# KerkDovan/univer-ocr

Hardware: NVIDIA B200
Metric: my_model inference images/sec (page tiles through Monochrome->Paragraph + Line + Char forward) (higher is better)
Workload: dtype tf32/f32

## Files before the change

univer_ocr_b200/csrc/conv_pair_rows_tc.cu:

```cuda
#include <cuda.h>

#include "conv_common.cuh"
#include "tc_ptx.cuh"

namespace uocr {

int make_tmap_plain_tf32(CUtensorMap* map, const void* base, int rank, const uint64_t* dims,
                         const uint64_t* strides_bytes, const uint32_t* box);

namespace {

constexpr int PR_THREADS = 672;
constexpr int PR_RING = 8;
constexpr int PR_SLOT = 2048;
constexpr int PR_OUT = 246;
constexpr int PR_TSLOTS = 4;
constexpr int PR_LAG = 2;

struct PairRowsParams {
    const float* w1; const float* b1; const float* w2; const float* b2; float* y;
    int N, H, W;
    int xt, nb, rb, npair;
    int total;
    float alpha1, alpha2;
};

struct __align__(128) PairRowsSmem {
    float ring[(PR_RING + 1) * PR_SLOT / 4];
    float ones[128 * 4];
    float b1[2][10 * 64 * 4];
    float b2[4][256];
    float xch[2][2][2];
    uint64_t full[PR_RING], empty[PR_RING];
    uint64_t hfull[PR_TSLOTS], a2full[PR_TSLOTS], zfull[PR_TSLOTS], zempty[PR_TSLOTS];
    uint64_t drain;
    uint32_t tmem;
};

struct WorkUnit {
    int y0, rows;
    int t, n0, n1;
    int S, c0;
};

__device__ __forceinline__ WorkUnit pr_decode(const PairRowsParams& p, int w) {
    WorkUnit u;
    const int pi = w % p.npair;
    const int rest = w / p.npair;
    u.t = rest % p.xt;
    const int b = rest / p.xt;
    u.y0 = b * p.rb;
    u.rows = min(p.rb, p.H - u.y0);
    u.n0 = 2 * pi;
    u.n1 = 2 * pi + 1;
    u.c0 = (u.t & 1) ? 5 : 3;
    u.S = PR_OUT * u.t - 1 - u.c0;
    return u;
}

__device__ __forceinline__ void pr_wait(uint32_t bar, uint32_t parity) { mbar_wait(bar, parity); }

__device__ __forceinline__ void pr_ld16(uint32_t taddr, float* v) {
    uint32_t* r = reinterpret_cast<uint32_t*>(v);
    tc_ld16_nowait(taddr, r);
}
__device__ __forceinline__ void pr_st16(uint32_t taddr, const float* v) {
    tc_st16_nowait(taddr, reinterpret_cast<const uint32_t*>(v));
}

__device__ __forceinline__ bool pr_elect() {
    uint32_t pred;
    asm volatile("{\n\t.reg .pred p;\n\telect.sync _|p, 0xffffffff;\n\tselp.u32 %0, 1, 0, p;\n\t}" : "=r"(pred));
    return pred != 0;
}

__device__ void pr_producer(const PairRowsParams& p, const CUtensorMap* map, PairRowsSmem& sm) {
    const uint32_t ring = smem_u32(sm.ring);
    uint32_t ut = 0;
    for (int w = blockIdx.x; w < p.total; w += gridDim.x) {
        const WorkUnit u = pr_decode(p, w);
        const int nin = u.rows + 4;
        for (int r = 0; r < nin; ++r, ++ut) {
            const uint32_t slot = ut % PR_RING;
            pr_wait(smem_u32(&sm.empty[slot]), ((ut / PR_RING) & 1u) ^ 1u);
            if (pr_elect()) {
                const uint32_t bar = smem_u32(&sm.full[slot]);
                const bool mirror = slot == 0;
                mbar_arrive_expect_tx(bar, mirror ? 2u * PR_SLOT : (uint32_t)PR_SLOT);
                const int y = u.y0 - 2 + r;
                const uint32_t dst = ring + slot * PR_SLOT;
                tma_load_3d(dst, map, bar, u.S, y, u.n0);
                tma_load_3d(dst + 1024, map, bar, u.S, y, u.n1);
                if (mirror) {
                    const uint32_t dst2 = ring + PR_RING * PR_SLOT;
                    tma_load_3d(dst2, map, bar, u.S, y, u.n0);
                    tma_load_3d(dst2 + 1024, map, bar, u.S, y, u.n1);
                }
            }
            __syncwarp();
        }
    }
}

__device__ __forceinline__ void pr_conv2(PairRowsSmem& sm, uint32_t tmem, int j, uint32_t kv, uint64_t db2_0,
                                         uint64_t db2_1, uint32_t id16) {
    const uint32_t par = (kv / PR_TSLOTS) & 1u;
    pr_wait(smem_u32(&sm.a2full[j]), par);
    pr_wait(smem_u32(&sm.zempty[j]), par ^ 1u);
    tc_fence_after();
    if (pr_elect()) {
        const uint32_t base = tmem + 128u * (uint32_t)j;
#pragma unroll
        for (int f = 0; f < 4; ++f) {
            tc_mma_tf32_ts(base + 64u + 16u * f, base + 16u * f, db2_0 + 64u * f, id16, 0);
            tc_mma_tf32_ts(base + 64u + 16u * f, base + 16u * f + 8u, db2_1 + 64u * f, id16, 1);
        }
        tc_commit(smem_u32(&sm.zfull[j]));
    }
    __syncwarp();
}

__device__ void pr_mma(const PairRowsParams& p, PairRowsSmem& sm, uint32_t tmem, int j) {
    const uint32_t ring = smem_u32(sm.ring), ones = smem_u32(sm.ones), sb2 = smem_u32(sm.b2);
    const uint32_t id64 = (1u << 4) | (2u << 7) | (2u << 10) | ((64u >> 3) << 17) | ((128u >> 4) << 24);
    const uint32_t id16 = (1u << 4) | (2u << 7) | (2u << 10) | ((16u >> 3) << 17) | ((128u >> 4) << 24);
    const uint64_t da_row = make_kmajor_nosw_desc(0, 16, 128);
    const uint64_t da_pair = make_kmajor_nosw_desc(0, PR_SLOT, 128);
    const uint64_t da_bias = make_kmajor_nosw_desc(0, 0, 128);
    const uint64_t db2_0 = make_kmajor_nosw_desc(sb2, 256, 128), db2_1 = make_kmajor_nosw_desc(sb2 + 512, 256, 128);
    const uint32_t d1 = tmem + 128u * (uint32_t)j;
    uint32_t ut = 0, kv = 0;
    bool pending = false;
    uint32_t pkv = 0;
    for (int w = blockIdx.x; w < p.total; w += gridDim.x) {
        const WorkUnit u = pr_decode(p, w);
        const uint32_t sb1 = smem_u32(sm.b1[u.c0 == 5 ? 1 : 0]);
        const uint64_t db_ky0 = make_kmajor_nosw_desc(sb1 + 0 * 1024, 1024, 128);
        const uint64_t db_ky1 = make_kmajor_nosw_desc(sb1 + 3 * 1024, 1024, 128);
        const uint64_t db_ky2 = make_kmajor_nosw_desc(sb1 + 6 * 1024, 1024, 128);
        const uint64_t db_c2 = make_kmajor_nosw_desc(sb1 + 2 * 1024, 3 * 1024, 128);
        const uint64_t db_bias = make_kmajor_nosw_desc(sb1 + 8 * 1024, 1024, 128);
        const int nh = u.rows + 2;
        const int r_lo = u.y0 == 0 ? 1 : 0, r_hi = min(nh, p.H - u.y0 + 1);
        const int below = (j == 0 && r_hi < nh) ? r_hi : nh;
        int first = r_lo + (int)((uint32_t)(j - (int)(kv & 3u)) & 3u);
        if (first >= r_hi) first = below;
        int r = (j == 0 && r_lo == 1) ? 0 : first;
        while (r < nh) {
            const bool valid = r >= r_lo && r < r_hi;
            const uint32_t kvr = kv + (uint32_t)(r - r_lo);
            int r_next = r < r_lo ? first : (valid ? r + 4 : nh);
            if (valid && r_next >= r_hi) r_next = below;
            if (pending) {
                pr_conv2(sm, tmem, j, pkv, db2_0, db2_1, id16);
                pending = false;
            }
            const uint32_t u0 = ut + (uint32_t)r;
            const uint32_t s0 = u0 % PR_RING, s1 = (u0 + 1u) % PR_RING, s2 = (u0 + 2u) % PR_RING;
            const uint32_t e0 = smem_u32(&sm.empty[s0]), e1 = smem_u32(&sm.empty[s1]), e2 = smem_u32(&sm.empty[s2]);
            pr_wait(smem_u32(&sm.full[s0]), (u0 / PR_RING) & 1u);
            pr_wait(smem_u32(&sm.full[s1]), ((u0 + 1u) / PR_RING) & 1u);
            pr_wait(smem_u32(&sm.full[s2]), ((u0 + 2u) / PR_RING) & 1u);
            tc_fence_after();
            if (pr_elect()) {
                if (valid) {
                    const uint64_t a0 = (uint64_t)((ring + s0 * PR_SLOT) >> 4);
                    const uint64_t a1 = (uint64_t)((ring + s1 * PR_SLOT) >> 4);
                    const uint64_t a2 = (uint64_t)((ring + s2 * PR_SLOT) >> 4);
                    tc_mma_tf32(d1, da_row + a0, db_ky0, id64, 0);
                    tc_mma_tf32(d1, da_row + a1, db_ky1, id64, 1);
                    tc_mma_tf32(d1, da_row + a2, db_ky2, id64, 1);
                    tc_mma_tf32(d1, da_pair + a0 + 2u, db_c2, id64, 1);
                    tc_mma_tf32(d1, da_bias + (a2 + 2u) + ((uint64_t)((ones >> 4) - (uint32_t)(a2 + 2u)) << 16), db_bias,
                                id64, 1);
                    tc_commit(smem_u32(&sm.hfull[j]));
                    tc_commit(e0);
                    tc_commit(e1);
                    tc_commit(e2);
                } else {
                    mbar_arrive(e0);
                    mbar_arrive(e1);
                    mbar_arrive(e2);
                }
                if (r == 0) { mbar_arrive(e0); mbar_arrive(e0); mbar_arrive(e1); }
                if (r == nh - 1) { mbar_arrive(e1); mbar_arrive(e2); mbar_arrive(e2); }
            }
            __syncwarp();
            if (valid) { pending = true; pkv = kvr; }
            r = r_next;
        }
        kv += (uint32_t)(r_hi - r_lo);
        ut += (uint32_t)(nh + 2);
    }
    if (pending) pr_conv2(sm, tmem, j, pkv, db2_0, db2_1, id16);
    if (pr_elect()) tc_commit(smem_u32(&sm.drain));
    __syncwarp();
    pr_wait(smem_u32(&sm.drain), 0);
}

__device__ __forceinline__ int pr_tap(int f, int n) {
    int kx = -1, ky = 0;
    if (f == 0)      { if (n < 6) { kx = n / 3; ky = n % 3; } else if (n >= 8 && n < 11) { kx = 2; ky = n - 8; } }
    else if (f == 1) { if (n < 6) { kx = 1 + n / 3; ky = n % 3; } else if (n >= 8 && n < 11) { kx = 0; ky = n - 8; } }
    else if (f == 2) { if (n < 3) { kx = 2; ky = n; } else if (n >= 8 && n < 14) { kx = (n - 8) / 3; ky = (n - 8) % 3; } }
    else             { if (n < 3) { kx = 0; ky = n; } else if (n >= 8 && n < 14) { kx = 1 + (n - 8) / 3; ky = (n - 8) % 3; } }
    return kx < 0 ? -1 : ky * 3 + kx;
}

template <bool LEAKY>
__device__ void pr_act(const PairRowsParams& p, PairRowsSmem& sm, uint32_t tmem, int q, int type, int lane) {
    const uint32_t tl = tmem + ((uint32_t)(q * 32) << 16) + 32u * (uint32_t)type;
    const int j = (q & 1) * 32 + lane;
    const uint32_t hbar = smem_u32(&sm.hfull[0]), abar = smem_u32(&sm.a2full[0]);
    const uint32_t alpha_bits = __float_as_uint(p.alpha1);
    uint32_t k = 0;
    for (int w = blockIdx.x; w < p.total; w += gridDim.x) {
        const WorkUnit u = pr_decode(p, w);
        const int x0 = u.S + u.c0 + 4 * j + 2 * type;
        const bool in0 = x0 >= 0 && x0 < p.W, in1 = x0 + 1 >= 0 && x0 + 1 < p.W;
        const bool edge = !(in0 && in1);
        const int r_lo = u.y0 == 0 ? 1 : 0, r_hi = min(u.rows + 2, p.H - u.y0 + 1);
        for (int r = r_lo; r < r_hi; ++r, ++k) {
            const uint32_t s = k & 3u;
            pr_wait(hbar + 8u * s, (k >> 2) & 1u);
            tc_fence_after();
            uint32_t h[32];
            tc_ld16_nowait(tl + 128u * s, h);
            tc_ld16_nowait(tl + 128u * s + 16u, h + 16);
            tc_wait_ld();
            if (LEAKY) {
#pragma unroll
                for (int c = 0; c < 32; c += 2) {
                    uint32_t t0, t1;
                    asm("{\n\t.reg .b64 x, y, r;\n\tmov.b64 x, {%2, %3};\n\tmov.b64 y, {%4, %4};\n\t"
                        "mul.rn.f32x2 r, x, y;\n\tmov.b64 {%0, %1}, r;\n\t}"
                        : "=r"(t0), "=r"(t1) : "r"(h[c]), "r"(h[c + 1]), "r"(alpha_bits));
                    h[c] = __float_as_uint(fmaxf(__uint_as_float(h[c]), __uint_as_float(t0)));
                    h[c + 1] = __float_as_uint(fmaxf(__uint_as_float(h[c + 1]), __uint_as_float(t1)));
                }
            }
            if (edge) {
#pragma unroll
                for (int c = 0; c < 16; ++c) {
                    if (!in0) h[c] = 0u;
                    if (!in1) h[16 + c] = 0u;
                }
            }
            tc_st16_nowait(tl + 128u * s, h);
            tc_st16_nowait(tl + 128u * s + 16u, h + 16);
            tc_wait_st();
            tc_fence_before();
            mbar_arrive(abar + 8u * s);
        }
    }
}

struct EpiState {
    float acc[3][6];
};

__device__ __forceinline__ void pr_ld4(uint32_t taddr, float* v) {
    uint32_t* r = reinterpret_cast<uint32_t*>(v);
    asm volatile("tcgen05.ld.sync.aligned.32x32b.x4.b32 {%0, %1, %2, %3}, [%4];"
                 : "=r"(r[0]), "=r"(r[1]), "=r"(r[2]), "=r"(r[3]) : "r"(taddr) : "memory");
}

struct EpiCtx {
    uint32_t tl;
    uint32_t zfull, zempty, xch;
    float bias2, alpha2;
    int barrier_id;
    bool send, recv, st0, st1;
};

__device__ __forceinline__ float pr_sigmoid(float v) {
    float e, r;
    asm("ex2.approx.ftz.f32 %0, %1;" : "=f"(e) : "f"(v * -1.4426950408889634f));
    asm("rcp.approx.ftz.f32 %0, %1;" : "=f"(r) : "f"(1.f + e));
    return r;
}

template <int PH, bool SIGMOID, int TYPE>
__device__ __forceinline__ void pr_epi_row(const EpiCtx& c, EpiState& st, uint32_t& k, uint32_t& xcount, bool valid,
                                           bool emit, float* __restrict__ yrow) {
    if (valid) {
        float za[8], zb[8], zc[4], zd[4];
        const uint32_t s = k & 3u;
        pr_wait(c.zfull + 8u * s, (k >> 2) & 1u);
        tc_fence_after();
        const uint32_t zt = c.tl + 128u * s;
        if (TYPE == 0) {
            tc_ld8_nowait(zt + 0u, reinterpret_cast<uint32_t*>(za));
            tc_ld8_nowait(zt + 16u, reinterpret_cast<uint32_t*>(zb));
            pr_ld4(zt + 32u, zc);
            pr_ld4(zt + 48u, zd);
        } else {
            pr_ld4(zt + 8u, zc);
            pr_ld4(zt + 24u, zd);
            tc_ld8_nowait(zt + 40u, reinterpret_cast<uint32_t*>(za));
            tc_ld8_nowait(zt + 56u, reinterpret_cast<uint32_t*>(zb));
        }
        tc_wait_ld();
        tc_fence_before();
        mbar_arrive(c.zempty + 8u * s);
        ++k;
#define PR_ACC(V, SRC, OFF)                                \
        st.acc[(PH + 2) % 3][V] = SRC[OFF];                \
        st.acc[(PH + 1) % 3][V] += SRC[OFF + 1];           \
        st.acc[PH][V] += SRC[OFF + 2];
        if (TYPE == 0) {
            PR_ACC(0, za, 0) PR_ACC(1, za, 3) PR_ACC(2, zb, 0) PR_ACC(3, zb, 3) PR_ACC(4, zc, 0) PR_ACC(5, zd, 0)
        } else {
            PR_ACC(0, zc, 0) PR_ACC(1, zd, 0) PR_ACC(2, za, 0) PR_ACC(3, za, 3) PR_ACC(4, zb, 0) PR_ACC(5, zb, 3)
        }
#undef PR_ACC
    } else {
#pragma unroll
        for (int v = 0; v < 6; ++v) st.acc[(PH + 2) % 3][v] = 0.f;
    }
    if (!emit) return;
    const uint32_t slot = c.xch + 4u * (xcount++ & 1u);
    float nb;
    if (TYPE == 0) nb = __shfl_up_sync(0xffffffffu, st.acc[PH][5], 1);
    else nb = __shfl_down_sync(0xffffffffu, st.acc[PH][0], 1);
    if (c.send) asm volatile("st.shared.f32 [%0], %1;" ::"r"(slot), "f"(TYPE == 0 ? st.acc[PH][5] : st.acc[PH][0]) : "memory");
    asm volatile("bar.sync %0, 64;" ::"r"(c.barrier_id) : "memory");
    if (c.recv) asm volatile("ld.shared.f32 %0, [%1];" : "=f"(nb) : "r"(slot) : "memory");
    float v0, v1;
    if (TYPE == 0) {
        v0 = (nb + st.acc[PH][1]) + (st.acc[PH][3] + c.bias2);
        v1 = (st.acc[PH][0] + st.acc[PH][2]) + (st.acc[PH][4] + c.bias2);
    } else {
        v0 = (st.acc[PH][1] + st.acc[PH][3]) + (st.acc[PH][5] + c.bias2);
        v1 = (st.acc[PH][2] + st.acc[PH][4]) + (nb + c.bias2);
    }
    if (SIGMOID) {
        v0 = pr_sigmoid(v0);
        v1 = pr_sigmoid(v1);
    } else if (c.alpha2 != 1.f) {
        v0 = v0 >= 0.f ? v0 : v0 * c.alpha2;
        v1 = v1 >= 0.f ? v1 : v1 * c.alpha2;
    }
    if (c.st0) yrow[0] = v0;
    if (c.st1) yrow[1] = v1;
}

template <bool SIGMOID, int TYPE>
__device__ void pr_epi(const PairRowsParams& p, PairRowsSmem& sm, uint32_t tmem, int q, int lane) {
    const int tile = q >> 1;
    const int j = (q & 1) * 32 + lane;
    EpiCtx c;
    c.tl = tmem + ((uint32_t)(q * 32) << 16) + 64u;
    c.zfull = smem_u32(&sm.zfull[0]);
    c.zempty = smem_u32(&sm.zempty[0]);
    c.xch = smem_u32(&sm.xch[TYPE][tile][0]);
    c.bias2 = __ldg(p.b2);
    c.alpha2 = p.alpha2;
    c.barrier_id = 1 + 2 * TYPE + tile;
    c.send = TYPE == 0 ? ((q & 1) == 0 && lane == 31) : ((q & 1) == 1 && lane == 0);
    c.recv = TYPE == 0 ? ((q & 1) == 1 && lane == 0) : ((q & 1) == 0 && lane == 31);
    uint32_t k = 0, xcount = 0;
    for (int w = blockIdx.x; w < p.total; w += gridDim.x) {
        const WorkUnit u = pr_decode(p, w);
        const int n = tile ? u.n1 : u.n0;
        const int x0 = u.S + u.c0 + 4 * j + 2 * TYPE;
        const int hp = 4 * j + 2 * TYPE;
        c.st0 = n < p.N && hp >= 1 && hp <= PR_OUT && x0 < p.W;
        c.st1 = n < p.N && hp + 1 >= 1 && hp + 1 <= PR_OUT && x0 + 1 < p.W;
        EpiState st;
#pragma unroll
        for (int a = 0; a < 3; ++a)
#pragma unroll
            for (int v = 0; v < 6; ++v) st.acc[a][v] = 0.f;
        const int nh = u.rows + 2;
        const int r_lo = u.y0 == 0 ? 1 : 0, r_hi = min(nh, p.H - u.y0 + 1);
        float* yrow = p.y + ((int64_t)(n < p.N ? n : 0) * p.H + (u.y0 - 2)) * (int64_t)p.W + x0;
#define PR_ROW(PH, R)                                                                                              \
        pr_epi_row<PH, SIGMOID, TYPE>(c, st, k, xcount, (R) >= r_lo && (R) < r_hi, (R) >= 2, yrow);                \
        yrow += p.W;
        for (int r = 0; r < nh; r += 3) {
            PR_ROW(0, r)
            if (r + 1 < nh) { PR_ROW(1, r + 1) }
            if (r + 2 < nh) { PR_ROW(2, r + 2) }
        }
#undef PR_ROW
    }
}

template <bool LEAKY, bool SIGMOID>
__global__ void __launch_bounds__(PR_THREADS, 1) conv3x3_pair_rows_kernel(const __grid_constant__ CUtensorMap map_x,
                                                                          const PairRowsParams p) {
    __shared__ PairRowsSmem sm;
    const int tid = threadIdx.x, lane = tid & 31;
    const int warp = __shfl_sync(0xffffffffu, tid >> 5, 0);

    for (int i = tid; i < 2 * 10 * 64 * 4; i += PR_THREADS) {
        const int var = i / 2560, rest = i % 2560;
        const int kc = rest / 256, n = (rest % 256) >> 2, e = rest & 3;
        const int c0 = var ? 5 : 3, f = n >> 4, c = n & 15;
        float v = 0.f;
        if (kc < 9) {
            const int ky = kc / 3, fr = 4 * (kc % 3) + e;
            const int kx = fr - (c0 + f) + 1;
            if (kx >= 0 && kx < 3) v = __ldg(p.w1 + (ky * 3 + kx) * 16 + c);
        } else if (e == 0) {
            v = __ldg(p.b1 + c);
        }
        sm.b1[var][kc * 256 + n * 4 + e] = round_tf32(v * (1.f + 1.f / 2048.f));
    }
    for (int i = tid; i < 4 * 256; i += PR_THREADS) {
        const int f = i >> 8, rest = i & 255;
        const int kq = rest >> 6, n = (rest & 63) >> 2, kk = rest & 3;
        const int tap = pr_tap(f, n);
        sm.b2[f][rest] = tap >= 0 ? round_tf32(__ldg(p.w2 + tap * 16 + kq * 4 + kk)) : 0.f;
    }
    for (int i = tid; i < 512; i += PR_THREADS) sm.ones[i] = (i & 3) == 0 ? 1.f : 0.f;
    if (tid == 0) {
        for (int s = 0; s < PR_RING; ++s) {
            mbar_init(smem_u32(&sm.full[s]), 1);
            mbar_init(smem_u32(&sm.empty[s]), 3);
        }
        for (int s = 0; s < PR_TSLOTS; ++s) {
            mbar_init(smem_u32(&sm.hfull[s]), 1);
            mbar_init(smem_u32(&sm.a2full[s]), 256);
            mbar_init(smem_u32(&sm.zfull[s]), 1);
            mbar_init(smem_u32(&sm.zempty[s]), 256);
        }
        mbar_init(smem_u32(&sm.drain), PR_TSLOTS);
        asm volatile("fence.mbarrier_init.release.cluster;" ::: "memory");
    }
    asm volatile("fence.proxy.async.shared::cta;" ::: "memory");
    if (warp == 17) {
        asm volatile("tcgen05.alloc.cta_group::1.sync.aligned.shared::cta.b32 [%0], %1;"
                     ::"r"(smem_u32(&sm.tmem)), "r"(512u) : "memory");
        asm volatile("tcgen05.relinquish_alloc_permit.cta_group::1.sync.aligned;" ::: "memory");
    }
    tc_fence_before();
    __syncthreads();
    tc_fence_after();
    const uint32_t tmem = sm.tmem;

    if (warp == 16) {
        pr_producer(p, &map_x, sm);
    } else if (warp >= 17) {
        pr_mma(p, sm, tmem, warp - 17);
    } else if (warp < 8) {
        pr_act<LEAKY>(p, sm, tmem, warp & 3, warp >> 2, lane);
    } else if (warp < 12) {
        pr_epi<SIGMOID, 0>(p, sm, tmem, warp & 3, lane);
    } else {
        pr_epi<SIGMOID, 1>(p, sm, tmem, warp & 3, lane);
    }

    tc_fence_before();
    __syncthreads();
    if (warp == 17) {
        tc_fence_after();
        asm volatile("tcgen05.dealloc.cta_group::1.sync.aligned.b32 %0, %1;" ::"r"(tmem), "r"(512u) : "memory");
    }
}

}

int conv3x3_pair_rows(const float* x, const float* w1, const float* b1, const float* w2, const float* b2, float* y,
                      int64_t n, int64_t h, int64_t w, int c1, int act1, float alpha1, int act2, float alpha2,
                      cudaStream_t st) {
    if (c1 != 16 || w % 4 || w < 8 || n > 0x3fffffff) return UOCR_ERR_UNSUPPORTED;
    if ((reinterpret_cast<uintptr_t>(x) & 15) != 0) return UOCR_ERR_UNSUPPORTED;
    const bool leaky = act1 == UOCR_ACT_LEAKY;
    if (!(act1 == UOCR_ACT_NONE || (leaky && alpha1 >= 0.f && alpha1 <= 1.f))) return UOCR_ERR_UNSUPPORTED;
    static int sms = 0;
    if (!sms) {
        int dev = 0;
        cudaGetDevice(&dev);
        cudaDeviceGetAttribute(&sms, cudaDevAttrMultiProcessorCount, dev);
        if (sms <= 0) sms = 148;
    }
    PairRowsParams p{};
    p.w1 = w1; p.b1 = b1; p.w2 = w2; p.b2 = b2; p.y = y;
    p.N = (int)n; p.H = (int)h; p.W = (int)w;
    p.xt = (int)ceil_div(w, PR_OUT);
    p.npair = (int)ceil_div(n, 2);
    int best_nb = 1;
    double best_cost = 1e300;
    for (int nb = 1; nb <= 32 && nb <= h; ++nb) {
        const int64_t rb = ceil_div(h, nb);
        const int64_t units = (int64_t)ceil_div(h, rb) * p.xt * p.npair;
        const double cost = (double)ceil_div(units, sms) * (double)(rb + 2 + 6);
        if (cost < best_cost) { best_cost = cost; best_nb = nb; }
    }
    p.rb = (int)ceil_div(h, best_nb);
    p.nb = (int)ceil_div(h, p.rb);
    const int64_t total = (int64_t)p.nb * p.xt * p.npair;
    if (total > 0x7fffffff) return UOCR_ERR_UNSUPPORTED;
    p.total = (int)total;
    p.alpha1 = alpha1;
    p.alpha2 = act2 == UOCR_ACT_LEAKY ? alpha2 : 1.f;
    CUtensorMap map;
    const uint64_t dims[3] = {(uint64_t)w, (uint64_t)h, (uint64_t)n};
    const uint64_t strides[2] = {(uint64_t)w * 4, (uint64_t)w * h * 4};
    const uint32_t box[3] = {256, 1, 1};
    int rc = make_tmap_plain_tf32(&map, x, 3, dims, strides, box);
    if (rc) return rc;
    unsigned grid = (unsigned)(total < sms ? total : sms);
    { const char* e = getenv("UOCR_PAIR_ROWS_GRID"); if (e && atoi(e) > 0 && (unsigned)atoi(e) < grid) grid = (unsigned)atoi(e); }
    if (act2 == UOCR_ACT_SIGMOID) {
        if (leaky) conv3x3_pair_rows_kernel<true, true><<<grid, PR_THREADS, 0, st>>>(map, p);
        else conv3x3_pair_rows_kernel<false, true><<<grid, PR_THREADS, 0, st>>>(map, p);
    } else {
        if (leaky) conv3x3_pair_rows_kernel<true, false><<<grid, PR_THREADS, 0, st>>>(map, p);
        else conv3x3_pair_rows_kernel<false, false><<<grid, PR_THREADS, 0, st>>>(map, p);
    }
    UOCR_LAUNCHED("conv3x3_pair_rows");
    return UOCR_OK;
}

}
```

Measured before the change: 171,200.

## Split activation warps by row parity instead of by column half

Previously each activation warp handled one 32-column half (type) of every row's TMEM tile, so two warp groups each arrived on every row slot. Now each warp processes all 64 columns of alternating rows, chosen by the row index parity combined with type, and the a2full barrier expects 128 arrivals instead of 256. This halves the barrier waits and arrivals per warp and lets two rows' activations proceed concurrently in different warps. The cost is longer per-row latency, since a single warp does twice the TMEM load/store work before the MMA can consume that slot.

```diff
diff --git a/univer_ocr_b200/csrc/conv_pair_rows_tc.cu b/univer_ocr_b200/csrc/conv_pair_rows_tc.cu
--- a/univer_ocr_b200/csrc/conv_pair_rows_tc.cu
+++ b/univer_ocr_b200/csrc/conv_pair_rows_tc.cu
@@ -208,50 +208,58 @@
 }
 
 template <bool LEAKY>
+__device__ __forceinline__ void pr_act_half(uint32_t taddr, uint32_t alpha_bits, bool in_a, bool in_b) {
+    uint32_t h[32];
+    tc_ld16_nowait(taddr, h);
+    tc_ld16_nowait(taddr + 16u, h + 16);
+    tc_wait_ld();
+    if (LEAKY) {
+#pragma unroll
+        for (int c = 0; c < 32; c += 2) {
+            uint32_t t0, t1;
+            asm("{\n\t.reg .b64 x, y, r;\n\tmov.b64 x, {%2, %3};\n\tmov.b64 y, {%4, %4};\n\t"
+                "mul.rn.f32x2 r, x, y;\n\tmov.b64 {%0, %1}, r;\n\t}"
+                : "=r"(t0), "=r"(t1) : "r"(h[c]), "r"(h[c + 1]), "r"(alpha_bits));
+            h[c] = __float_as_uint(fmaxf(__uint_as_float(h[c]), __uint_as_float(t0)));
+            h[c + 1] = __float_as_uint(fmaxf(__uint_as_float(h[c + 1]), __uint_as_float(t1)));
+        }
+    }
+    if (!(in_a && in_b)) {
+#pragma unroll
+        for (int c = 0; c < 16; ++c) {
+            if (!in_a) h[c] = 0u;
+            if (!in_b) h[16 + c] = 0u;
+        }
+    }
+    tc_st16_nowait(taddr, h);
+    tc_st16_nowait(taddr + 16u, h + 16);
+}
+
+template <bool LEAKY>
 __device__ void pr_act(const PairRowsParams& p, PairRowsSmem& sm, uint32_t tmem, int q, int type, int lane) {
-    const uint32_t tl = tmem + ((uint32_t)(q * 32) << 16) + 32u * (uint32_t)type;
+    const uint32_t tl = tmem + ((uint32_t)(q * 32) << 16);
     const int j = (q & 1) * 32 + lane;
     const uint32_t hbar = smem_u32(&sm.hfull[0]), abar = smem_u32(&sm.a2full[0]);
     const uint32_t alpha_bits = __float_as_uint(p.alpha1);
     uint32_t k = 0;
     for (int w = blockIdx.x; w < p.total; w += gridDim.x) {
         const WorkUnit u = pr_decode(p, w);
-        const int x0 = u.S + u.c0 + 4 * j + 2 * type;
-        const bool in0 = x0 >= 0 && x0 < p.W, in1 = x0 + 1 >= 0 && x0 + 1 < p.W;
-        const bool edge = !(in0 && in1);
+        const int x0 = u.S + u.c0 + 4 * j;
+        bool in[4];
+#pragma unroll
+        for (int f = 0; f < 4; ++f) in[f] = x0 + f >= 0 && x0 + f < p.W;
         const int r_lo = u.y0 == 0 ? 1 : 0, r_hi = min(u.rows + 2, p.H - u.y0 + 1);
-        for (int r = r_lo; r < r_hi; ++r, ++k) {
-            const uint32_t s = k & 3u;
-            pr_wait(hbar + 8u * s, (k >> 2) & 1u);
+        for (int r = r_lo + (int)((k ^ (uint32_t)type) & 1u); r < r_hi; r += 2) {
+            const uint32_t kr = k + (uint32_t)(r - r_lo), s = kr & 3u;
+            pr_wait(hbar + 8u * s, (kr >> 2) & 1u);
             tc_fence_after();
-            uint32_t h[32];
-            tc_ld16_nowait(tl + 128u * s, h);
-            tc_ld16_nowait(tl + 128u * s + 16u, h + 16);
-            tc_wait_ld();
-            if (LEAKY) {
-#pragma unroll
-                for (int c = 0; c < 32; c += 2) {
-                    uint32_t t0, t1;
-                    asm("{\n\t.reg .b64 x, y, r;\n\tmov.b64 x, {%2, %3};\n\tmov.b64 y, {%4, %4};\n\t"
-                        "mul.rn.f32x2 r, x, y;\n\tmov.b64 {%0, %1}, r;\n\t}"
-                        : "=r"(t0), "=r"(t1) : "r"(h[c]), "r"(h[c + 1]), "r"(alpha_bits));
-                    h[c] = __float_as_uint(fmaxf(__uint_as_float(h[c]), __uint_as_float(t0)));
-                    h[c + 1] = __float_as_uint(fmaxf(__uint_as_float(h[c + 1]), __uint_as_float(t1)));
-                }
-            }
-            if (edge) {
-#pragma unroll
-                for (int c = 0; c < 16; ++c) {
-                    if (!in0) h[c] = 0u;
-                    if (!in1) h[16 + c] = 0u;
-                }
-            }
-            tc_st16_nowait(tl + 128u * s, h);
-            tc_st16_nowait(tl + 128u * s + 16u, h + 16);
+            pr_act_half<LEAKY>(tl + 128u * s, alpha_bits, in[0], in[1]);
+            pr_act_half<LEAKY>(tl + 128u * s + 32u, alpha_bits, in[2], in[3]);
             tc_wait_st();
             tc_fence_before();
             mbar_arrive(abar + 8u * s);
         }
+        k += (uint32_t)(r_hi - r_lo);
     }
 }
 
@@ -422,7 +430,7 @@
         }
         for (int s = 0; s < PR_TSLOTS; ++s) {
             mbar_init(smem_u32(&sm.hfull[s]), 1);
-            mbar_init(smem_u32(&sm.a2full[s]), 256);
+            mbar_init(smem_u32(&sm.a2full[s]), 128);
             mbar_init(smem_u32(&sm.zfull[s]), 1);
             mbar_init(smem_u32(&sm.zempty[s]), 256);
         }
```

Measured after the change: 171,600 (median of 6 runs). About the same (+0.3%).

## Process conv rows in pairs with two MMA warps and double-buffered TMEM slots

Applied to the files above, without the earlier changes.

Restructures the fused two-layer conv pipeline so each MMA warp processes two output rows per step (two pairs of TMEM slots of 256 columns) instead of four MMA warps each handling one row, cutting the thread count from 672 to 608. The activation and epilogue warps now load, transform and consume two rows per barrier handshake, which halves the number of mbarrier waits and commits per row. Empty-barrier counts and ring-slot release logic are reworked to match. This trades per-row parallelism across MMA warps for fewer synchronisations, and carries a risk of subtle ring/barrier accounting bugs at tile edges.

```diff
diff --git a/univer_ocr_b200/csrc/conv_pair_rows_tc.cu b/univer_ocr_b200/csrc/conv_pair_rows_tc.cu
--- a/univer_ocr_b200/csrc/conv_pair_rows_tc.cu
+++ b/univer_ocr_b200/csrc/conv_pair_rows_tc.cu
@@ -10,12 +10,12 @@
 
 namespace {
 
-constexpr int PR_THREADS = 672;
+constexpr int PR_THREADS = 608;
 constexpr int PR_RING = 8;
 constexpr int PR_SLOT = 2048;
 constexpr int PR_OUT = 246;
-constexpr int PR_TSLOTS = 4;
-constexpr int PR_LAG = 2;
+constexpr int PR_PSLOTS = 2;
+constexpr uint32_t PR_PCOLS = 256;
 
 struct PairRowsParams {
     const float* w1; const float* b1; const float* w2; const float* b2; float* y;
@@ -32,7 +32,7 @@
     float b2[4][256];
     float xch[2][2][2];
     uint64_t full[PR_RING], empty[PR_RING];
-    uint64_t hfull[PR_TSLOTS], a2full[PR_TSLOTS], zfull[PR_TSLOTS], zempty[PR_TSLOTS];
+    uint64_t hfull[PR_PSLOTS], a2full[PR_PSLOTS], zfull[PR_PSLOTS], zempty[PR_PSLOTS];
     uint64_t drain;
     uint32_t tmem;
 };
@@ -102,25 +102,31 @@
     }
 }
 
-__device__ __forceinline__ void pr_conv2(PairRowsSmem& sm, uint32_t tmem, int j, uint32_t kv, uint64_t db2_0,
-                                         uint64_t db2_1, uint32_t id16) {
-    const uint32_t par = (kv / PR_TSLOTS) & 1u;
-    pr_wait(smem_u32(&sm.a2full[j]), par);
-    pr_wait(smem_u32(&sm.zempty[j]), par ^ 1u);
+__device__ __forceinline__ void pr_conv2(PairRowsSmem& sm, uint32_t tmem, int s, uint32_t kp, bool va, bool vb,
+                                         uint64_t db2_0, uint64_t db2_1, uint32_t id16) {
+    const uint32_t par = (kp / PR_PSLOTS) & 1u;
+    pr_wait(smem_u32(&sm.a2full[s]), par);
+    pr_wait(smem_u32(&sm.zempty[s]), par ^ 1u);
     tc_fence_after();
     if (pr_elect()) {
-        const uint32_t base = tmem + 128u * (uint32_t)j;
-#pragma unroll
-        for (int f = 0; f < 4; ++f) {
-            tc_mma_tf32_ts(base + 64u + 16u * f, base + 16u * f, db2_0 + 64u * f, id16, 0);
-            tc_mma_tf32_ts(base + 64u + 16u * f, base + 16u * f + 8u, db2_1 + 64u * f, id16, 1);
-        }
-        tc_commit(smem_u32(&sm.zfull[j]));
+        const uint32_t base = tmem + PR_PCOLS * (uint32_t)s;
+#pragma unroll
+        for (int h = 0; h < 2; ++h) {
+            if (h == 0 ? va : vb) {
+                const uint32_t a = base + 64u * h, z = base + 128u + 64u * h;
+#pragma unroll
+                for (int f = 0; f < 4; ++f) {
+                    tc_mma_tf32_ts(z + 16u * f, a + 16u * f, db2_0 + 64u * f, id16, 0);
+                    tc_mma_tf32_ts(z + 16u * f, a + 16u * f + 8u, db2_1 + 64u * f, id16, 1);
+                }
+            }
+        }
+        tc_commit(smem_u32(&sm.zfull[s]));
     }
     __syncwarp();
 }
 
-__device__ void pr_mma(const PairRowsParams& p, PairRowsSmem& sm, uint32_t tmem, int j) {
+__device__ void pr_mma(const PairRowsParams& p, PairRowsSmem& sm, uint32_t tmem, int ps) {
     const uint32_t ring = smem_u32(sm.ring), ones = smem_u32(sm.ones), sb2 = smem_u32(sm.b2);
     const uint32_t id64 = (1u << 4) | (2u << 7) | (2u << 10) | ((64u >> 3) << 17) | ((128u >> 4) << 24);
     const uint32_t id16 = (1u << 4) | (2u << 7) | (2u << 10) | ((16u >> 3) << 17) | ((128u >> 4) << 24);
@@ -128,10 +134,10 @@
     const uint64_t da_pair = make_kmajor_nosw_desc(0, PR_SLOT, 128);
     const uint64_t da_bias = make_kmajor_nosw_desc(0, 0, 128);
     const uint64_t db2_0 = make_kmajor_nosw_desc(sb2, 256, 128), db2_1 = make_kmajor_nosw_desc(sb2 + 512, 256, 128);
-    const uint32_t d1 = tmem + 128u * (uint32_t)j;
-    uint32_t ut = 0, kv = 0;
-    bool pending = false;
-    uint32_t pkv = 0;
+    const uint32_t d1 = tmem + PR_PCOLS * (uint32_t)ps;
+    uint32_t ut = 0, kp = 0;
+    bool pending = false, pva = false, pvb = false;
+    uint32_t pkp = 0;
     for (int w = blockIdx.x; w < p.total; w += gridDim.x) {
         const WorkUnit u = pr_decode(p, w);
         const uint32_t sb1 = smem_u32(sm.b1[u.c0 == 5 ? 1 : 0]);
@@ -142,57 +148,62 @@
         const uint64_t db_bias = make_kmajor_nosw_desc(sb1 + 8 * 1024, 1024, 128);
         const int nh = u.rows + 2;
         const int r_lo = u.y0 == 0 ? 1 : 0, r_hi = min(nh, p.H - u.y0 + 1);
-        const int below = (j == 0 && r_hi < nh) ? r_hi : nh;
-        int first = r_lo + (int)((uint32_t)(j - (int)(kv & 3u)) & 3u);
-        if (first >= r_hi) first = below;
-        int r = (j == 0 && r_lo == 1) ? 0 : first;
-        while (r < nh) {
-            const bool valid = r >= r_lo && r < r_hi;
-            const uint32_t kvr = kv + (uint32_t)(r - r_lo);
-            int r_next = r < r_lo ? first : (valid ? r + 4 : nh);
-            if (valid && r_next >= r_hi) r_next = below;
+        for (int r = 0; r < nh; r += 2) {
+            const bool present = r < r_hi;
+            if ((kp & 1u) != (uint32_t)ps) {
+                kp += present ? 1u : 0u;
+                continue;
+            }
+            const bool va = r >= r_lo && r < r_hi, vb = r + 1 < r_hi;
+            const bool two = r + 1 < nh;
             if (pending) {
-                pr_conv2(sm, tmem, j, pkv, db2_0, db2_1, id16);
+                pr_conv2(sm, tmem, ps, pkp, pva, pvb, db2_0, db2_1, id16);
                 pending = false;
             }
             const uint32_t u0 = ut + (uint32_t)r;
-            const uint32_t s0 = u0 % PR_RING, s1 = (u0 + 1u) % PR_RING, s2 = (u0 + 2u) % PR_RING;
-            const uint32_t e0 = smem_u32(&sm.empty[s0]), e1 = smem_u32(&sm.empty[s1]), e2 = smem_u32(&sm.empty[s2]);
-            pr_wait(smem_u32(&sm.full[s0]), (u0 / PR_RING) & 1u);
-            pr_wait(smem_u32(&sm.full[s1]), ((u0 + 1u) / PR_RING) & 1u);
-            pr_wait(smem_u32(&sm.full[s2]), ((u0 + 2u) / PR_RING) & 1u);
+            uint32_t e[4], a[4];
+#pragma unroll
+            for (int i = 0; i < 4; ++i) {
+                const uint32_t ui = u0 + (uint32_t)i, si = ui % PR_RING;
+                e[i] = smem_u32(&sm.empty[si]);
+                a[i] = (ring + si * PR_SLOT) >> 4;
+                if (i < 3 || two) pr_wait(smem_u32(&sm.full[si]), (ui / PR_RING) & 1u);
+            }
             tc_fence_after();
             if (pr_elect()) {
-                if (valid) {
-                    const uint64_t a0 = (uint64_t)((ring + s0 * PR_SLOT) >> 4);
-                    const uint64_t a1 = (uint64_t)((ring + s1 * PR_SLOT) >> 4);
-                    const uint64_t a2 = (uint64_t)((ring + s2 * PR_SLOT) >> 4);
-                    tc_mma_tf32(d1, da_row + a0, db_ky0, id64, 0);
-                    tc_mma_tf32(d1, da_row + a1, db_ky1, id64, 1);
-                    tc_mma_tf32(d1, da_row + a2, db_ky2, id64, 1);
-                    tc_mma_tf32(d1, da_pair + a0 + 2u, db_c2, id64, 1);
-                    tc_mma_tf32(d1, da_bias + (a2 + 2u) + ((uint64_t)((ones >> 4) - (uint32_t)(a2 + 2u)) << 16), db_bias,
-                                id64, 1);
-                    tc_commit(smem_u32(&sm.hfull[j]));
-                    tc_commit(e0);
-                    tc_commit(e1);
-                    tc_commit(e2);
+#pragma unroll
+                for (int h = 0; h < 2; ++h) {
+                    if (h == 0 ? va : vb) {
+                        const uint32_t d = d1 + 64u * h;
+                        const uint64_t a0 = a[h], a1 = a[h + 1], a2 = a[h + 2];
+                        tc_mma_tf32(d, da_row + a0, db_ky0, id64, 0);
+                        tc_mma_tf32(d, da_row + a1, db_ky1, id64, 1);
+                        tc_mma_tf32(d, da_row + a2, db_ky2, id64, 1);
+                        tc_mma_tf32(d, da_pair + a0 + 2u, db_c2, id64, 1);
+                        tc_mma_tf32(d, da_bias + (a2 + 2u) + ((uint64_t)((ones >> 4) - (uint32_t)(a2 + 2u)) << 16),
+                                    db_bias, id64, 1);
+                    }
+                }
+                if (present) {
+                    tc_commit(smem_u32(&sm.hfull[ps]));
+                    tc_commit(e[0]);
+                    tc_commit(e[1]);
+                    tc_commit(e[2]);
+                    if (two) tc_commit(e[3]);
                 } else {
-                    mbar_arrive(e0);
-                    mbar_arrive(e1);
-                    mbar_arrive(e2);
+                    mbar_arrive(e[0]);
+                    mbar_arrive(e[1]);
+                    mbar_arrive(e[2]);
                 }
-                if (r == 0) { mbar_arrive(e0); mbar_arrive(e0); mbar_arrive(e1); }
-                if (r == nh - 1) { mbar_arrive(e1); mbar_arrive(e2); mbar_arrive(e2); }
+                if (r == 0) { mbar_arrive(e[0]); mbar_arrive(e[1]); }
+                if (r + 2 >= nh) { mbar_arrive(e[2]); if (two) mbar_arrive(e[3]); }
             }
             __syncwarp();
-            if (valid) { pending = true; pkv = kvr; }
-            r = r_next;
-        }
-        kv += (uint32_t)(r_hi - r_lo);
+            if (present) { pending = true; pkp = kp; pva = va; pvb = vb; ++kp; }
+        }
         ut += (uint32_t)(nh + 2);
     }
-    if (pending) pr_conv2(sm, tmem, j, pkv, db2_0, db2_1, id16);
+    if (pending) pr_conv2(sm, tmem, ps, pkp, pva, pvb, db2_0, db2_1, id16);
     if (pr_elect()) tc_commit(smem_u32(&sm.drain));
     __syncwarp();
     pr_wait(smem_u32(&sm.drain), 0);
@@ -219,18 +230,20 @@
         const int x0 = u.S + u.c0 + 4 * j + 2 * type;
         const bool in0 = x0 >= 0 && x0 < p.W, in1 = x0 + 1 >= 0 && x0 + 1 < p.W;
         const bool edge = !(in0 && in1);
-        const int r_lo = u.y0 == 0 ? 1 : 0, r_hi = min(u.rows + 2, p.H - u.y0 + 1);
-        for (int r = r_lo; r < r_hi; ++r, ++k) {
-            const uint32_t s = k & 3u;
-            pr_wait(hbar + 8u * s, (k >> 2) & 1u);
+        const int r_hi = min(u.rows + 2, p.H - u.y0 + 1);
+        for (int r = 0; r < r_hi; r += 2, ++k) {
+            const uint32_t s = k & 1u, ts = tl + PR_PCOLS * s;
+            pr_wait(hbar + 8u * s, (k >> 1) & 1u);
             tc_fence_after();
-            uint32_t h[32];
-            tc_ld16_nowait(tl + 128u * s, h);
-            tc_ld16_nowait(tl + 128u * s + 16u, h + 16);
+            uint32_t h[64];
+            tc_ld16_nowait(ts, h);
+            tc_ld16_nowait(ts + 16u, h + 16);
+            tc_ld16_nowait(ts + 64u, h + 32);
+            tc_ld16_nowait(ts + 80u, h + 48);
             tc_wait_ld();
             if (LEAKY) {
 #pragma unroll
-                for (int c = 0; c < 32; c += 2) {
+                for (int c = 0; c < 64; c += 2) {
                     uint32_t t0, t1;
                     asm("{\n\t.reg .b64 x, y, r;\n\tmov.b64 x, {%2, %3};\n\tmov.b64 y, {%4, %4};\n\t"
                         "mul.rn.f32x2 r, x, y;\n\tmov.b64 {%0, %1}, r;\n\t}"
@@ -242,12 +255,14 @@
             if (edge) {
 #pragma unroll
                 for (int c = 0; c < 16; ++c) {
-                    if (!in0) h[c] = 0u;
-                    if (!in1) h[16 + c] = 0u;
+                    if (!in0) { h[c] = 0u; h[32 + c] = 0u; }
+                    if (!in1) { h[16 + c] = 0u; h[48 + c] = 0u; }
                 }
             }
-            tc_st16_nowait(tl + 128u * s, h);
-            tc_st16_nowait(tl + 128u * s + 16u, h + 16);
+            tc_st16_nowait(ts, h);
+            tc_st16_nowait(ts + 16u, h + 16);
+            tc_st16_nowait(ts + 64u, h + 32);
+            tc_st16_nowait(ts + 80u, h + 48);
             tc_wait_st();
             tc_fence_before();
             mbar_arrive(abar + 8u * s);
@@ -268,8 +283,7 @@
 struct EpiCtx {
     uint32_t tl;
     uint32_t zfull, zempty, xch;
-    float bias2, alpha2;
-    int barrier_id;
+    float bias2;
     bool send, recv, st0, st1;
 };
 
@@ -280,51 +294,51 @@
     return r;
 }
 
-template <int PH, bool SIGMOID, int TYPE>
-__device__ __forceinline__ void pr_epi_row(const EpiCtx& c, EpiState& st, uint32_t& k, uint32_t& xcount, bool valid,
-                                           bool emit, float* __restrict__ yrow) {
+template <int PH, int TYPE>
+__device__ __forceinline__ void pr_acc_row(EpiState& st, bool valid, uint32_t zt) {
     if (valid) {
+#define PR_ACC(V, SRC, OFF)                                \
+        st.acc[(PH + 2) % 3][V] = SRC[OFF];                \
+        st.acc[(PH + 1) % 3][V] += SRC[OFF + 1];           \
+        st.acc[PH][V] += SRC[OFF + 2];
         float za[8], zb[8], zc[4], zd[4];
-        const uint32_t s = k & 3u;
-        pr_wait(c.zfull + 8u * s, (k >> 2) & 1u);
-        tc_fence_after();
-        const uint32_t zt = c.tl + 128u * s;
         if (TYPE == 0) {
             tc_ld8_nowait(zt + 0u, reinterpret_cast<uint32_t*>(za));
             tc_ld8_nowait(zt + 16u, reinterpret_cast<uint32_t*>(zb));
+            tc_wait_ld();
             pr_ld4(zt + 32u, zc);
             pr_ld4(zt + 48u, zd);
+            PR_ACC(0, za, 0) PR_ACC(1, za, 3) PR_ACC(2, zb, 0) PR_ACC(3, zb, 3)
+            tc_wait_ld();
+            PR_ACC(4, zc, 0) PR_ACC(5, zd, 0)
         } else {
             pr_ld4(zt + 8u, zc);
             pr_ld4(zt + 24u, zd);
             tc_ld8_nowait(zt + 40u, reinterpret_cast<uint32_t*>(za));
+            tc_wait_ld();
             tc_ld8_nowait(zt + 56u, reinterpret_cast<uint32_t*>(zb));
-        }
-        tc_wait_ld();
-        tc_fence_before();
-        mbar_arrive(c.zempty + 8u * s);
-        ++k;
-#define PR_ACC(V, SRC, OFF)                                \
-        st.acc[(PH + 2) % 3][V] = SRC[OFF];                \
-        st.acc[(PH + 1) % 3][V] += SRC[OFF + 1];           \
-        st.acc[PH][V] += SRC[OFF + 2];
-        if (TYPE == 0) {
-            PR_ACC(0, za, 0) PR_ACC(1, za, 3) PR_ACC(2, zb, 0) PR_ACC(3, zb, 3) PR_ACC(4, zc, 0) PR_ACC(5, zd, 0)
-        } else {
-            PR_ACC(0, zc, 0) PR_ACC(1, zd, 0) PR_ACC(2, za, 0) PR_ACC(3, za, 3) PR_ACC(4, zb, 0) PR_ACC(5, zb, 3)
+            PR_ACC(0, zc, 0) PR_ACC(1, zd, 0) PR_ACC(2, za, 0) PR_ACC(3, za, 3)
+            tc_wait_ld();
+            PR_ACC(4, zb, 0) PR_ACC(5, zb, 3)
         }
 #undef PR_ACC
     } else {
 #pragma unroll
         for (int v = 0; v < 6; ++v) st.acc[(PH + 2) % 3][v] = 0.f;
     }
-    if (!emit) return;
+}
+
+template <int PH, bool SIGMOID, int TYPE>
+__device__ __forceinline__ void pr_emit(const EpiCtx& c, const EpiState& st, uint32_t& xcount, float alpha2,
+                                        float* __restrict__ yrow) {
     const uint32_t slot = c.xch + 4u * (xcount++ & 1u);
     float nb;
     if (TYPE == 0) nb = __shfl_up_sync(0xffffffffu, st.acc[PH][5], 1);
     else nb = __shfl_down_sync(0xffffffffu, st.acc[PH][0], 1);
     if (c.send) asm volatile("st.shared.f32 [%0], %1;" ::"r"(slot), "f"(TYPE == 0 ? st.acc[PH][5] : st.acc[PH][0]) : "memory");
-    asm volatile("bar.sync %0, 64;" ::"r"(c.barrier_id) : "memory");
+    uint32_t tid;
+    asm volatile("mov.u32 %0, %%tid.x;" : "=r"(tid));
+    asm volatile("bar.sync %0, 64;" ::"r"(1u + 2u * TYPE + ((tid >> 6) & 1u)) : "memory");
     if (c.recv) asm volatile("ld.shared.f32 %0, [%1];" : "=f"(nb) : "r"(slot) : "memory");
     float v0, v1;
     if (TYPE == 0) {
@@ -337,12 +351,33 @@
     if (SIGMOID) {
         v0 = pr_sigmoid(v0);
         v1 = pr_sigmoid(v1);
-    } else if (c.alpha2 != 1.f) {
-        v0 = v0 >= 0.f ? v0 : v0 * c.alpha2;
-        v1 = v1 >= 0.f ? v1 : v1 * c.alpha2;
+    } else if (alpha2 != 1.f) {
+        v0 = v0 >= 0.f ? v0 : v0 * alpha2;
+        v1 = v1 >= 0.f ? v1 : v1 * alpha2;
     }
     if (c.st0) yrow[0] = v0;
     if (c.st1) yrow[1] = v1;
+}
+
+template <int PA, bool SIGMOID, int TYPE>
+__device__ __forceinline__ void pr_epi_pair(const EpiCtx& c, EpiState& st, uint32_t& k, uint32_t& xcount, bool va,
+                                            bool vb, bool two, bool ea, bool eb, int W, float alpha2,
+                                            float* __restrict__ yrow) {
+    constexpr int PB = (PA + 1) % 3;
+    const uint32_t s = k & 1u, zt = c.tl + PR_PCOLS * s;
+    if (va || vb) {
+        pr_wait(c.zfull + 8u * s, (k >> 1) & 1u);
+        tc_fence_after();
+    }
+    pr_acc_row<PA, TYPE>(st, va, zt);
+    if (ea) pr_emit<PA, SIGMOID, TYPE>(c, st, xcount, alpha2, yrow);
+    if (two) pr_acc_row<PB, TYPE>(st, vb, zt + 64u);
+    if (va || vb) {
+        tc_fence_before();
+        mbar_arrive(c.zempty + 8u * s);
+        ++k;
+    }
+    if (eb) pr_emit<PB, SIGMOID, TYPE>(c, st, xcount, alpha2, yrow + W);
 }
 
 template <bool SIGMOID, int TYPE>
@@ -350,13 +385,11 @@
     const int tile = q >> 1;
     const int j = (q & 1) * 32 + lane;
     EpiCtx c;
-    c.tl = tmem + ((uint32_t)(q * 32) << 16) + 64u;
+    c.tl = tmem + ((uint32_t)(q * 32) << 16) + 128u;
     c.zfull = smem_u32(&sm.zfull[0]);
     c.zempty = smem_u32(&sm.zempty[0]);
     c.xch = smem_u32(&sm.xch[TYPE][tile][0]);
     c.bias2 = __ldg(p.b2);
-    c.alpha2 = p.alpha2;
-    c.barrier_id = 1 + 2 * TYPE + tile;
     c.send = TYPE == 0 ? ((q & 1) == 0 && lane == 31) : ((q & 1) == 1 && lane == 0);
     c.recv = TYPE == 0 ? ((q & 1) == 1 && lane == 0) : ((q & 1) == 0 && lane == 31);
     uint32_t k = 0, xcount = 0;
@@ -375,15 +408,16 @@
         const int nh = u.rows + 2;
         const int r_lo = u.y0 == 0 ? 1 : 0, r_hi = min(nh, p.H - u.y0 + 1);
         float* yrow = p.y + ((int64_t)(n < p.N ? n : 0) * p.H + (u.y0 - 2)) * (int64_t)p.W + x0;
-#define PR_ROW(PH, R)                                                                                              \
-        pr_epi_row<PH, SIGMOID, TYPE>(c, st, k, xcount, (R) >= r_lo && (R) < r_hi, (R) >= 2, yrow);                \
-        yrow += p.W;
-        for (int r = 0; r < nh; r += 3) {
-            PR_ROW(0, r)
-            if (r + 1 < nh) { PR_ROW(1, r + 1) }
-            if (r + 2 < nh) { PR_ROW(2, r + 2) }
-        }
-#undef PR_ROW
+#define PR_PAIR(PA, R)                                                                                             \
+        pr_epi_pair<PA, SIGMOID, TYPE>(c, st, k, xcount, (R) >= r_lo && (R) < r_hi, (R) + 1 < r_hi, (R) + 1 < nh,  \
+                                       (R) >= 2, (R) >= 1 && (R) + 1 < nh, p.W, p.alpha2, yrow);                             \
+        yrow += 2 * (int64_t)p.W;
+        for (int r = 0; r < nh; r += 6) {
+            PR_PAIR(0, r)
+            if (r + 2 < nh) { PR_PAIR(2, r + 2) }
+            if (r + 4 < nh) { PR_PAIR(1, r + 4) }
+        }
+#undef PR_PAIR
     }
 }
 
@@ -418,15 +452,15 @@
     if (tid == 0) {
         for (int s = 0; s < PR_RING; ++s) {
             mbar_init(smem_u32(&sm.full[s]), 1);
-            mbar_init(smem_u32(&sm.empty[s]), 3);
-        }
-        for (int s = 0; s < PR_TSLOTS; ++s) {
+            mbar_init(smem_u32(&sm.empty[s]), 2);
+        }
+        for (int s = 0; s < PR_PSLOTS; ++s) {
             mbar_init(smem_u32(&sm.hfull[s]), 1);
             mbar_init(smem_u32(&sm.a2full[s]), 256);
             mbar_init(smem_u32(&sm.zfull[s]), 1);
             mbar_init(smem_u32(&sm.zempty[s]), 256);
         }
-        mbar_init(smem_u32(&sm.drain), PR_TSLOTS);
+        mbar_init(smem_u32(&sm.drain), PR_PSLOTS);
         asm volatile("fence.mbarrier_init.release.cluster;" ::: "memory");
     }
     asm volatile("fence.proxy.async.shared::cta;" ::: "memory");
@@ -454,9 +488,12 @@
 
     tc_fence_before();
     __syncthreads();
-    if (warp == 17) {
+    uint32_t tid_end;
+    asm volatile("mov.u32 %0, %%tid.x;" : "=r"(tid_end));
+    if (tid_end >> 5 == 17) {
         tc_fence_after();
-        asm volatile("tcgen05.dealloc.cta_group::1.sync.aligned.b32 %0, %1;" ::"r"(tmem), "r"(512u) : "memory");
+        asm volatile("tcgen05.dealloc.cta_group::1.sync.aligned.b32 %0, %1;"
+                     ::"r"(*reinterpret_cast<volatile uint32_t*>(&sm.tmem)), "r"(512u) : "memory");
     }
 }
 
```

Result: no change. 171,000 before, 169,500 after, median of 6 (-0.9%).
